# pangenome/poasta

Hardware: AMD Instinct MI355X
Metric: Gcells/sec (aligned bases/sec in config), gap-affine POA alignment, 1k-node POA x 10k x 1 kbp queries per GPU (higher is better)
Workload: dtype u16

## Files before the change

include/poasta_amd.h:

```cpp
#ifndef POASTA_AMD_H
#define POASTA_AMD_H

#include <stdint.h>

#ifdef __cplusplus
extern "C" {
#endif

#define POA_NONE 0xFFFFFFFFu
#define POA_SCORE_UNVISITED 0xFFFFFFFFu

#define POA_OK 0
#define POA_ERR_INVALID_ARG (-1)
#define POA_ERR_NOT_A_DAG (-2)
#define POA_ERR_NO_DEVICE (-3)
#define POA_ERR_HIP (-4)
#define POA_ERR_CAPACITY (-5)
#define POA_ERR_OUT_OF_MEMORY (-6)
#define POA_ERR_UNSUPPORTED (-7)

#define POA_FLAG_AMBIGUOUS 0x01u
#define POA_FLAG_START_QUIRK 0x02u
#define POA_FLAG_REF_PANIC 0x04u
#define POA_FLAG_SHORT_QUERY 0x08u
// ... 241 lines not shown
int poa_scoreset_workspace_bytes(poa_scoreset_t* s, uint64_t* bytes);
void poa_scoreset_destroy(poa_scoreset_t* s);
int poa_score_pairs(const poa_graph_t* const* graphs, uint32_t n_graphs, const poa_costs_t* costs, const poa_config_t* cfg,
                    uint32_t n_queries, const uint8_t* qseq, const uint64_t* qoff, uint64_t n_pairs, const uint32_t* pair_query,
                    const uint32_t* pair_graph, uint32_t* score, uint32_t* flags, poa_stats_t* stats, int device);
int poa_score_pairs_2piece(const poa_graph_t* const* graphs, uint32_t n_graphs, const poa_costs2_t* costs, const poa_config_t* cfg,
                           uint32_t n_queries, const uint8_t* qseq, const uint64_t* qoff, uint64_t n_pairs,
                           const uint32_t* pair_query, const uint32_t* pair_graph, uint32_t* score, uint32_t* flags,
                           poa_stats_t* stats, int device);

#ifdef __cplusplus
}
#endif
#include "poasta_amd_scoreset_cap.h"
#include "poasta_amd_scoreset_best.h"
#endif
```

poasta_amd/_lib.py:

```python
import ctypes as C
import os
import subprocess

_HERE = os.path.dirname(os.path.abspath(__file__))
LIB_PATH = os.environ.get("POA_LIB_PATH") or os.path.join(_HERE, "libpoasta_amd.so")
CSRC = os.path.join(_HERE, "csrc")

POA_OK = 0
ERRORS = {-1: "POA_ERR_INVALID_ARG", -2: "POA_ERR_NOT_A_DAG", -3: "POA_ERR_NO_DEVICE", -4: "POA_ERR_HIP",
          -5: "POA_ERR_CAPACITY", -6: "POA_ERR_OUT_OF_MEMORY", -7: "POA_ERR_UNSUPPORTED"}
POA_NONE = 0xFFFFFFFF
FLAG_AMBIGUOUS, FLAG_START_QUIRK, FLAG_REF_PANIC, FLAG_SHORT_QUERY, FLAG_TRUNCATED, FLAG_EMPTY_GRAPH = 1, 2, 4, 8, 16, 32
FLAG_CAPPED = 0x80

EXPORTS = ["poa_version", "poa_last_error", "poa_device_count", "poa_graph_create", "poa_graph_destroy",
           "poa_graph_rows", "poa_graph_node_rows", "poa_graph_update", "poa_align_batch", "poa_align_batch_ex", "poa_align_batch_2piece", "poa_align_batch_2piece_ex", "poa_planes_2piece", "poa_release_cache", "poa_batch_create", "poa_batch_run",
           "poa_batch_run_ex",
           "poa_batch_fetch", "poa_batch_stats", "poa_batch_device_results", "poa_batch_fetch_search_counters", "poa_batch_last_layout", "poa_batch_band_info", "poa_batch_band_pair_info", "poa_batch_band_narrow_info", "poa_batch_last_launch", "poa_batch_fetch_planes", "poa_batch_fetch_compact", "poa_batch_destroy",
           "poa_batch_run_2piece", "poa_batch_fetch_planes_2piece",
           "poa_graph_sweep_slots", "poa_batch_create_ex", "poa_batch_workspace_bytes", "poa_graph_checkpoint_plan", "poa_graph_checkpoint_plan2",
           "poa_multi_footprint", "poa_multi_create", "poa_multi_run", "poa_multi_fetch", "poa_multi_stats", "poa_multi_device_results",
           "poa_multi_workspace_bytes", "poa_multi_destroy", "poa_align_multi",
           "poa_multi_footprint_2piece", "poa_multi_create_2piece", "poa_multi_run_2piece", "poa_align_multi_2piece",
           "poa_scoreset_footprint", "poa_scoreset_create", "poa_scoreset_run", "poa_scoreset_run_2piece", "poa_scoreset_fetch",
           "poa_scoreset_stats", "poa_scoreset_device_results", "poa_scoreset_workspace_bytes", "poa_scoreset_destroy",
           "poa_score_pairs", "poa_score_pairs_2piece",
           "poa_graph_sweep_checks"]
EXPORTS_SCORESET_CAP = ["poa_scoreset_run_capped", "poa_scoreset_run_2piece_capped", "poa_scoreset_fetch_swept"]
EXPORTS_SCORESET_BEST = ["poa_scoreset_run_best", "poa_scoreset_run_2piece_best", "poa_scoreset_fetch_best", "poa_scoreset_device_best",
                         "poa_score_best", "poa_score_best_2piece"]
CFG_BEST_PAIR_ORDER = 2


class PoaBest(C.Structure):
    _fields_ = [("pair", C.c_uint32), ("score", C.c_uint32), ("flags", C.c_uint32), ("second_score", C.c_uint32),
                ("n_within", C.c_uint32), ("reserved", C.c_uint32 * 3)]


class PoaCosts2(C.Structure):
    _fields_ = [("mismatch", C.c_uint8), ("gap_open1", C.c_uint8), ("gap_extend1", C.c_uint8), ("gap_open2", C.c_uint8),
                ("gap_extend2", C.c_uint8), ("wide_planes", C.c_uint8), ("reserved", C.c_uint8 * 2)]


class PoaCosts(C.Structure):
    _fields_ = [("mismatch", C.c_uint8), ("gap_open", C.c_uint8), ("gap_extend", C.c_uint8), ("reserved", C.c_uint8)]

# ... 13 lines not shown
             "WS_CHUNK_CAP", "WS_PROF", "PS_LANES", "PS_LEAN", "TIMING", "WS_ADAPT", "WS_REC", "CKPT_ROWS", "BAND", "BAND_DELTA", "BAND_PAIR", "CAP_STRIDE")
EXACT_IMPLS = {"lane": 1, "wave": 2, "flat": 3}


def tune_from_env(cfg=None, **overrides):
    vals = {}
    for i, k in enumerate(TUNE_KEYS):
        v = overrides.get(k.lower(), os.environ.get("POA_" + k))
        if v is None or v == "":
            continue
        vals[i] = EXACT_IMPLS[v] if (k == "EXACT_IMPL" and v in EXACT_IMPLS) else int(v)
    nv = overrides.get("band_narrow", os.environ.get("POA_BAND_NARROW"))
    if nv is not None and nv != "":
        i = TUNE_KEYS.index("BAND_PAIR")
        vals[i] = (min(vals[i], 1) if i in vals else 2) | ((2 if int(nv) else 1) << 2)
    if cfg is None:
        if not vals:
            return None
        cfg = PoaConfig()
    for i, v in vals.items():
        cfg.tune[i] = v + 1
    return cfg


BOUND_UNBOUNDED, BOUND_INCLUDED, BOUND_EXCLUDED = 0, 1, 2
SPAN_GLOBAL, SPAN_ENDS_FREE = 0, 1


MODE_DENSE, MODE_EXACT, MODE_HYBRID, MODE_SCORE, MODE_CHECKPOINT, MODE_CHECKPOINT2 = 0, 1, 2, 3, 4, 5
HEURISTIC_DIJKSTRA, HEURISTIC_MINGAP = 0, 1
# ... 6 lines not shown
                ("n_chunks", C.c_uint32), ("n_forward_launches", C.c_uint32), ("n_flagged", C.c_uint32),
                ("ms_forward", C.c_float), ("ms_traceback", C.c_float), ("ms_h2d", C.c_float), ("ms_d2h", C.c_float),
                ("ms_exact", C.c_float), ("n_exact", C.c_uint32), ("ms_total", C.c_float), ("n_runs", C.c_uint32)]

    def as_dict(self):
        return {k: getattr(self, k) for k, _ in self._fields_ }


class PoaError(RuntimeError):
    def __init__(self, code, msg):
        super().__init__("%s (%d): %s" % (ERRORS.get(code, "POA_ERR"), code, msg))
        self.code = code


def build(force=False):
    srcs = [os.path.join(CSRC, f) for f in os.listdir(CSRC)] + [os.path.join(_HERE, "..", "include", h) for h in ("poasta_amd.h", "poasta_amd_scoreset_cap.h", "poasta_amd_scoreset_best.h")]
    stale = not os.path.exists(LIB_PATH) or any(os.path.getmtime(s) > os.path.getmtime(LIB_PATH) for s in srcs)
    if force or stale:
        subprocess.check_call(["make", "-C", CSRC] + (["-B"] if force else []))
    return LIB_PATH


_lib = None


def lib():
    global _lib
    if _lib is not None:
        return _lib
    if not os.path.exists(LIB_PATH):
        raise ImportError("poasta_amd: %s is missing — build it with `python -c 'import __graft_entry__ as g; g.build()'` "
# ... 70 lines not shown
    L.poa_batch_stats.restype = C.c_int
    L.poa_batch_stats.argtypes = [vp, C.POINTER(PoaStats)]
    L.poa_batch_fetch_search_counters.restype = C.c_int
    L.poa_batch_fetch_search_counters.argtypes = [vp, vp]
    L.poa_batch_last_layout.restype = C.c_int
    L.poa_batch_last_layout.argtypes = [vp, vp]
    if hasattr(L, "poa_batch_band_info"):
        L.poa_batch_band_info.restype = C.c_int
        L.poa_batch_band_info.argtypes = [vp, vp]
    if hasattr(L, "poa_batch_band_pair_info"):
        L.poa_batch_band_pair_info.restype = C.c_int
        L.poa_batch_band_pair_info.argtypes = [vp, vp]
    if hasattr(L, "poa_batch_band_narrow_info"):
        L.poa_batch_band_narrow_info.restype = C.c_int
        L.poa_batch_band_narrow_info.argtypes = [vp, vp]
    if hasattr(L, "poa_batch_last_launch"):
        L.poa_batch_last_launch.restype = C.c_int
        L.poa_batch_last_launch.argtypes = [vp, C.c_uint32, vp]
    L.poa_batch_device_results.restype = C.c_int
    L.poa_batch_device_results.argtypes = [vp, C.POINTER(vp), C.POINTER(vp), C.POINTER(vp), C.POINTER(vp)]
    L.poa_batch_fetch_planes.restype = C.c_int
    L.poa_batch_fetch_planes.argtypes = [vp, C.c_uint32, vp, vp, vp]
    if hasattr(L, "poa_batch_fetch_compact"):
        L.poa_batch_fetch_compact.restype = C.c_int
        L.poa_batch_fetch_compact.argtypes = [vp, C.c_uint32, vp, vp, vp]
    L.poa_batch_run_2piece.restype = C.c_int
    L.poa_batch_run_2piece.argtypes = [vp, C.POINTER(PoaCosts2), C.POINTER(PoaConfig), vp]
    L.poa_batch_fetch_planes_2piece.restype = C.c_int
    L.poa_batch_fetch_planes_2piece.argtypes = [vp, C.c_uint32, vp, vp, vp, vp, vp]
    L.poa_batch_destroy.argtypes = [vp]
# ... 63 lines not shown
```

poasta_amd/aligner.py:

```python
import ctypes as C
import os

import numpy as np

from . import _lib
from .graph import FlatGraph, pack_queries


class GapAffine:

    def __init__(self, cost_mismatch, cost_gap_extend, cost_gap_open):
        for v in (cost_mismatch, cost_gap_extend, cost_gap_open):
            if not 0 <= int(v) <= 255:
                raise ValueError("GapAffine costs are u8")
        self.cost_mismatch, self.cost_gap_extend, self.cost_gap_open = int(cost_mismatch), int(cost_gap_extend), int(cost_gap_open)

    def mismatch(self):
        return self.cost_mismatch

    def gap_open(self):
        return self.cost_gap_open

    def gap_extend(self):
        return self.cost_gap_extend
# ... 313 lines not shown

    def band_info(self):
        out = (C.c_uint32 * 4)()
        _lib.check(_lib.lib().poa_batch_band_info(self.handle, out))
        return {"used": bool(out[0]), "banded": int(out[1]), "fell_back": int(out[2]), "min_d": int(out[3])}

    def band_pair_info(self):
        out = (C.c_uint32 * 4)()
        _lib.check(_lib.lib().poa_batch_band_pair_info(self.handle, out))
        return {"paired": int(out[0]), "single": int(out[1]), "rule_count": int(out[2]), "ran_paired": bool(out[3])}

    def band_narrow_info(self):
        out = (C.c_uint32 * 4)()
        _lib.check(_lib.lib().poa_batch_band_narrow_info(self.handle, out))
        return {"ran": int(out[0]), "certified": int(out[1]), "certified_512": int(out[2]), "chosen_by": (None, "rule", "override")[int(out[3])]}

    def launches(self):
        out = []
        while True:
            v = (C.c_uint32 * 8)()
            rc = _lib.lib().poa_batch_last_launch(self.handle, len(out), v)
            if rc == -1 and (out or self.n == 0):
                return out
            _lib.check(rc)
            out.append({"kernel": LAUNCH_KERNELS[v[0]], "quads": int(v[1]), "fuse": bool(v[2] & 1), "mw": bool(v[2] & 2),
                        "waves": int(v[3]), "code_fmt": int(v[4]), "tb_lanes": int(v[5]), "tb_depth": int(v[6]), "queries": int(v[7])})

    def device_results(self):
        ptrs = [C.c_void_p() for _ in range(4)]
        _lib.check(_lib.lib().poa_batch_device_results(self.handle, *[C.byref(p) for p in ptrs]))
# ... 423 lines not shown
```

poasta_amd/csrc/poa_dense_plan.cpp:

```cpp
#include "poa_dense_plan.hpp"

#include <algorithm>

namespace poa_amd {

uint64_t score_bound(uint64_t open, uint64_t extend, uint64_t n_open, uint64_t n_extend) { return open * n_open + extend * n_extend; }
bool u16_cells_suffice(uint64_t open, uint64_t extend, uint64_t n_open, uint64_t n_extend) {
    return score_bound(open, extend, n_open, n_extend) <= 65534;
}
bool planes32(const TuneView& T) { const int* pv = T.ptr(POA_TUNE_PLANES); return pv && *pv == 32; }

uint32_t mw_waves(uint32_t strips) {
    const uint32_t groups = (strips + DENSE_MW_MAX_WAVES - 1) / DENSE_MW_MAX_WAVES;
    return (strips + groups - 1) / groups;
}

bool pxmw_ok(const TuneView& T, uint32_t count, uint32_t max_pitch) {
    if (const int* v = T.ptr(POA_TUNE_PXMW)) return (*v) != 0;
    return (uint64_t)count * ((max_pitch + 1023) / 1024) >= 1024;
}

DenseRunPlan plan_dense_run(uint32_t gap_open, uint32_t gap_extend, uint64_t max_len, uint64_t min_path_nodes, uint32_t mode, bool want_full,
                            bool plan16_same, const TuneView& T) {
    DenseRunPlan R;
// ... 13 lines not shown
    R.plan = (R.narrow && mode == POA_MODE_DENSE && !plan16_same) ? (R.compact ? 2 : 1) : 0;
    R.spec_depth = 12;
    if (const int* sv = T.ptr(POA_TUNE_TB_DEPTH)) { const int v = (*sv); if (v >= 1 && v <= 64) R.spec_depth = (uint32_t)v; }
    R.tb_group = 0;
    if (const int* gv = T.ptr(POA_TUNE_TB_GROUP)) { const int v = (*gv); if (v == 8 || v == 16 || v == 32 || v == 64) R.tb_group = v; }
    R.fuse_tb = false;
    if (const int* fv = T.ptr(POA_TUNE_FUSE_TB)) R.fuse_tb = (*fv) != 0;
    R.quads_override = 0;
    if (const int* ov = T.ptr(POA_TUNE_FWD_QUADS)) R.quads_override = (*ov);
    R.want_band = mode == POA_MODE_DENSE && gap_extend > 0;
    if (const int* bv = T.ptr(POA_TUNE_BAND)) R.want_band = R.want_band && (*bv) != 0;
    R.band_cap = 0xFFFFFFFFu;
    if (const int* dv = T.ptr(POA_TUNE_BAND_DELTA)) R.band_cap = (*dv) > 0 ? (uint32_t)(*dv) : 0u;
    R.band_pair = -1;
    R.band_narrow = -1;
    if (const int* pv = T.ptr(POA_TUNE_BAND_PAIR)) {
        const int p = (*pv) & POA_BAND_PAIR_MASK, n = ((*pv) >> POA_BAND_NARROW_SHIFT) & 3;
        if (p != POA_BAND_PAIR_RULE) R.band_pair = p != 0 ? 1 : 0;
        if (n) R.band_narrow = n - 1;
    }
    return R;
}

constexpr uint32_t BAND_NARROW_MIN_SHARE = 4;
uint32_t band_narrow_class(uint32_t d_n, uint32_t L) {
    if (d_n < 4) return 2;
    return (uint64_t)BAND_NARROW_MIN_SHARE * (d_n - 4) >= L ? 0 : 1;
}
uint32_t band_narrow_pairs(const DenseRunPlan& R, bool pair_by_rule, uint32_t n_rule, uint32_t n_any) {
    if (R.band_narrow == 0) return 0;
    if (R.band_narrow > 0) return n_any;
    return pair_by_rule ? n_rule : 0;
}

DenseChunkPlan plan_dense_chunk(const DenseRunPlan& R, uint32_t count, uint32_t max_pitch, const TuneView& T) {
    uint32_t lk = POA_KERNEL_NONE, lq = 0, lwaves = 4, code_fmt = 0;
    bool lfuse = false, lmw = false;
    int mf = -1;
    const int quads_override = R.quads_override;
    if (R.narrow) {
        uint32_t quads = max_pitch <= 512 ? 1 : 2;
        if (quads_override == 1 || quads_override == 2) quads = (uint32_t)quads_override;
        if (R.relative) quads = 2;
        lk = R.compact && R.packed ? POA_KERNEL_PACKED : POA_KERNEL_FORWARD; lq = quads;
        if (R.compact && R.packed) {
            bool mw = max_pitch > 512 * quads;
            if (const int* mv = T.ptr(POA_TUNE_MW)) mw = mw && ((*mv) != 0 || R.relative);
            bool px = max_pitch <= 1024 && quads == 2 && (!R.fuse_tb || R.relative);
            if (const int* xv = T.ptr(POA_TUNE_PX)) px = (px && (*xv) != 0) || (px && R.relative);
            if (px) {
// ... 19 lines not shown
        if (mw) {
            const uint32_t s2 = (max_pitch + 511) / 512, s4 = (max_pitch + 1023) / 1024;
            const uint32_t g2 = (s2 + DENSE_MW_MAX_WAVES - 1) / DENSE_MW_MAX_WAVES, g4 = (s4 + 9) / 10;
            bool wide = 14 * g4 < 10 * g2 || (uint64_t)count * s4 >= 8192;
            if (quads_override == 4) wide = true;
            if (quads_override == 2) wide = false;
            lq = wide ? 4 : 2; lmw = true; lwaves = wide ? (s4 + g4 - 1) / g4 : (s2 + g2 - 1) / g2;
        } else lfuse = R.fuse_tb;
    }
    uint32_t ltb = 0, ldepth = R.spec_depth;
    if (!(R.fuse_tb && !R.relative && max_pitch <= 1024 && (!R.compact || R.packed))) {
        const int tbg = R.tb_group ? R.tb_group : (count <= 6144 ? 64 : (count <= 12288 ? 32 : 16));
        ltb = R.compact ? (uint32_t)tbg : 64u;
        if (R.compact && !T.ptr(POA_TUNE_TB_DEPTH)) ldepth = tbg == 16 ? 16u : 32u;
    }
    return {{lk, lq, (lfuse ? POA_LAUNCH_FUSE : 0u) | (lmw ? POA_LAUNCH_MW : 0u), lwaves, code_fmt, ltb, ldepth, count}, mf, lk == POA_KERNEL_BAND, ltb != 0};
}

}
```

poasta_amd/csrc/poa_dense_plan.hpp:

```cpp
#pragma once
#include <cstdint>

#include "../../include/poasta_amd.h"

struct TuneView {
    int val[POA_TUNE_COUNT]; bool set[POA_TUNE_COUNT];
    explicit TuneView(const poa_config_t* cfg) { for (int k = 0; k < POA_TUNE_COUNT; ++k) { set[k] = cfg && cfg->tune[k] != 0; val[k] = set[k] ? (int)cfg->tune[k] - 1 : 0; } }
    const int* ptr(int k) const { return set[k] ? &val[k] : nullptr; }
};

namespace poa_amd {
constexpr uint32_t DENSE_MW_MAX_WAVES = 16;
uint64_t score_bound(uint64_t open, uint64_t extend, uint64_t n_open, uint64_t n_extend);
bool u16_cells_suffice(uint64_t open, uint64_t extend, uint64_t n_open, uint64_t n_extend);
bool planes32(const TuneView& T);
uint32_t mw_waves(uint32_t strips);
bool pxmw_ok(const TuneView& T, uint32_t count, uint32_t max_pitch);

struct DenseRunPlan {
    uint64_t ub;
    bool narrow, compact, relative, packed;
    int plan;
    bool fuse_tb, want_band;
    int quads_override, band_pair, tb_group;
    int band_narrow;
    uint32_t band_cap, spec_depth;
};
DenseRunPlan plan_dense_run(uint32_t gap_open, uint32_t gap_extend, uint64_t max_len, uint64_t min_path_nodes, uint32_t mode, bool full_planes,
                            bool plan16_same, const TuneView& T);

struct DenseChunkPlan {
    uint32_t v[8];
    int mf;
    bool band;
    bool separate_tb;
};
DenseChunkPlan plan_dense_chunk(const DenseRunPlan& R, uint32_t count, uint32_t max_pitch, const TuneView& T);
uint32_t band_narrow_class(uint32_t d_n, uint32_t L);
uint32_t band_narrow_pairs(const DenseRunPlan& R, bool pair_by_rule, uint32_t n_rule, uint32_t n_any);
}
```

poasta_amd/csrc/poa_engine.hip:

```cpp
#include <hip/hip_runtime.h>

#include <algorithm>
#include <array>
#include <chrono>
#include <cstdio>
#include <cstdlib>
#include <cstring>
#include <map>
#include <memory>
#include <new>
#include <mutex>
#include <string>
#include <vector>

#include "../../include/poasta_amd.h"
#include "poa_graph.hpp"
#include "poa_exact_kernel.hpp"
#include "poa_wsearch.hpp"
#include "poa_fsearch.hpp"

#include "poa_dense_plan.hpp"
#include "poa_kernels.hpp"
#include "poa_forward_packed.hpp"
#include "poa_forward_px.hpp"
#include "poa_band_plan.hpp"
#include "poa_forward_band.hpp"
#include "poa_twopiece.hpp"
#include "poa_sweep_rows.hpp"
#include "poa_forward_sweep.hpp"
#include "poa_checkpoint.hpp"
#include "poa_checkpoint2.hpp"
#include "poa_multi_plan.hpp"
#include "poa_multi.hpp"
#include "poa_scoreset_plan.hpp"
#include "poa_scoreset.hpp"

using namespace poa_amd;
// ... 194 lines not shown
    CheckpointPlan ckpt_plan;
    uint32_t ckpt_slots = 0;
    bool ckpt2 = false;
    DevBuf<uint32_t> d_ck_snap_off, d_ck_snap_dst, d_ck_pred_src, d_ck_boundary;

    bool band_ready = false;
    uint32_t band_n_seg = 0;
    std::vector<uint32_t> h_band_cls, h_band_d;
    DevBuf<uint32_t> d_band_cls, d_band_d, d_band_base;
    DevBuf<uint32_t> d_band_list, d_band_count;
    std::vector<uint32_t> h_band_dn;
    DevBuf<uint32_t> d_band_dn, d_band_base_n, d_band_list_n;
    std::vector<uint32_t> h_band_order;
    std::vector<uint32_t> h_band_nnarrow_rule, h_band_nnarrow_any;
    uint32_t narrow_ran = 0, narrow_how = 0, narrow_chunks = 0;
    int band_pair_plan = -1;
    std::vector<uint32_t> h_band_npair;
    DevBuf<uint32_t> d_band_order;
    uint32_t pair_paired = 0, pair_single = 0;
    bool band_used = false;
    uint32_t band_queries = 0, band_min_d = 0, band_chunks = 0;
    std::vector<DenseChunkPlan> launches;

    std::vector<std::vector<hipEvent_t>> runs;
    std::vector<std::vector<hipEvent_t>> free_sets;
    bool ran = false;
    hipStream_t last_stream = nullptr;
    float ms_h2d = 0.f;

    ~poa_batch() {
// ... 348 lines not shown
    HIP_TRY(hipGetLastError());
    hipLaunchKernelGGL(poa_forward_band_kernel<true>, dim3(blocks), dim3(256), 0, stream, fp, bp);
    uint32_t min_d = 0xFFFFFFFFu;
    for (uint32_t i = ch.first; i < ch.first + ch.count; ++i) min_d = std::min(min_d, std::min(b->h_band_d[b->h_band_cls[i]], R.band_cap));
    for (uint32_t k = 0; k < 2 * n_narrow; ++k) min_d = std::min(min_d, std::min(b->h_band_dn[b->h_band_cls[b->h_band_order[ch.first + k]]], R.band_cap));
    b->band_min_d = b->band_used ? std::min(b->band_min_d, min_d) : min_d;
    b->band_used = true; b->band_queries += ch.count; b->band_chunks = (uint32_t)ci + 1;
    return POA_OK;
}

void launch_traceback(const DenseRunPlan& R, const DenseChunkPlan& c, const TbParams& tp, hipStream_t stream) {
    const uint32_t lanes = c.v[5], per_block = 256 / lanes;
    const dim3 grid((c.v[7] + per_block - 1) / per_block), block(256);
    TbParams tpg = tp;
    tpg.spec_depth = c.v[6];
    if (R.compact && lanes == 16) hipLaunchKernelGGL((poa_traceback_kernel<uint16_t, true, 16>), grid, block, 0, stream, tpg);
    else if (R.compact && lanes == 32) hipLaunchKernelGGL((poa_traceback_kernel<uint16_t, true, 32>), grid, block, 0, stream, tpg);
    else if (R.compact && lanes == 8) hipLaunchKernelGGL((poa_traceback_kernel<uint16_t, true, 8>), grid, block, 0, stream, tpg);
    else if (R.compact) hipLaunchKernelGGL((poa_traceback_kernel<uint16_t, true>), grid, block, 0, stream, tpg);
    else if (R.narrow) hipLaunchKernelGGL((poa_traceback_kernel<uint16_t, false>), grid, block, 0, stream, tp);
    else hipLaunchKernelGGL((poa_traceback_kernel<uint32_t, false>), grid, block, 0, stream, tp);
}

template <typename SearchParams>
void fill_search_params(SearchParams& sp, poa_batch* b, const ExactParams& ep, const TuneView& T) {
    sp.E = ep;
    sp.chunks = reinterpret_cast<ExU4*>(b->d_ex_pool.p);
    sp.chunk_cap = b->ex_pool_cap / BQ_CHUNK;
    if (const int* cv = T.ptr(POA_TUNE_WS_CHUNK_CAP)) { const int v = (*cv); if (v >= 1 && (uint32_t)v < sp.chunk_cap) sp.chunk_cap = (uint32_t)v; }
    sp.win = b->ex_win;
    sp.counters = b->d_ex_counters.p;
// ... 721 lines not shown
        if (rc != POA_OK) return rc;
    }
    RunFrame run;
    if (const int rc = run.open(b, "poa_batch_run: call poa_batch_stats/fetch at least every 256 runs")) return rc;
    const DenseRunPlan R = plan_dense_run(costs->gap_open, costs->gap_extend, b->max_len, fg.min_path_nodes, mode,
                                          cfg && (cfg->flags & POA_CFG_FULL_PLANES), b->plan16_same, T);
    if (const int rc = run.begin(stream, b->plan[R.plan].chunks.size())) return rc;
    b->prof_on = T.ptr(POA_TUNE_WS_PROF) != nullptr;
    b->last_mode = mode;
    b->two_piece = false;
    set_layout(b, R.narrow, R.compact, R.relative);
    b->launches.clear();
    b->band_used = false; b->band_queries = 0; b->band_min_d = 0; b->band_chunks = 0;
    b->pair_paired = 0; b->pair_single = 0;
    b->narrow_ran = 0; b->narrow_how = 0; b->narrow_chunks = 0;
    b->active_plan = R.plan;
    const poa_batch::Plan& PL = b->cur();
    if (b->n_queries == 0) return run.end_empty(true);
    if (R.want_band && !PL.chunks.empty()) {
        if (b->d_band_count.n < 3 * PL.chunks.size()) HIP_TRY(b->d_band_count.alloc(3 * PL.chunks.size()));
        HIP_TRY(hipMemsetAsync(b->d_band_count.p, 0, 3 * PL.chunks.size() * 4, stream));
    }
    for (size_t ci = 0; ci < PL.chunks.size(); ++ci) {
        const auto& ch = PL.chunks[ci];
        uint32_t max_pitch = 0;
        for (uint32_t i = ch.first; i < ch.first + ch.count; ++i) max_pitch = std::max(max_pitch, b->h_pitch[i]);
        const DenseChunkPlan C = plan_dense_chunk(R, ch.count, max_pitch, T);
        TbParams tp;
        tp.rows = b->d_rows.p; tp.pred_rows = b->d_pred_rows.p; tp.n_rows = fg.n;
        tp.start_row = fg.start_row; tp.end_row = fg.end_row;
        tp.first_query = ch.first; tp.n_queries = ch.count;
        tp.qseq = b->d_qseq.p; tp.qoff = b->d_qoff.p; tp.pitch = b->d_pitch.p; tp.plane_off = PL.d_off.p;
        tp.planes = b->d_planes.p; tp.scratch_off = b->d_scratch_off.p; tp.scratch = b->d_scratch.p;
        tp.score = b->d_score.p; tp.flags = b->d_flags.p; tp.n_pairs = b->d_npairs.p;
        tp.cost_x = costs->mismatch; tp.cost_o = costs->gap_open; tp.cost_e = costs->gap_extend;
        tp.spec_depth = R.spec_depth;
        tp.exact_pass = 0; tp.ex_status = nullptr; tp.ex_end = nullptr; tp.code_fmt = C.v[4];
        tp.row_depth = R.relative ? b->d_row_depth.p : nullptr;
        tp.d_slot = fg.d_slot.empty() ? nullptr : b->d_dslot.p; tp.pred_dslot = fg.d_slot.empty() ? nullptr : b->d_pred_dslot.p;
        FwdParams fp;
        fp.rows = b->d_rows.p; fp.pred_rows = b->d_pred_rows.p; fp.n_rows = fg.n;
        fp.first_query = ch.first; fp.n_queries = ch.count;
// ... 4 lines not shown
        fp.cost_doe = R.relative ? (uint32_t)costs->gap_open : fp.cost_oe;
        fp.cost_ie = R.relative ? 2u * fp.cost_e : fp.cost_e;
        fp.cost_ioe = R.relative ? fp.cost_oe + fp.cost_e : fp.cost_oe;
        fp.pred_k = R.relative ? b->d_pred_k.p : nullptr;
        fp.d_slot = fg.d_slot.empty() ? nullptr : b->d_dslot.p; fp.pred_dslot = fg.d_slot.empty() ? nullptr : b->d_pred_dslot.p;
        fp.pipeline_error = b->d_pipeline_error.p;
        if (C.mf >= 0) b->dense_derived_gaps = C.mf == 3;
        if (C.band) { if (const int rc = launch_band(b, ci, R, fp, stream)) return rc; }
        else launch_forward(R, C, fp, tp, stream);
        HIP_TRY(hipGetLastError());
        if (const int rc = run.mark()) return rc;

        if (C.separate_tb) {
            launch_traceback(R, C, tp, stream);
            HIP_TRY(hipGetLastError());
        }
        if (mode == POA_MODE_DENSE) b->launches.push_back(C);
        if (const int rc = run.mark()) return rc;

        if (mode != POA_MODE_DENSE) {
            if (const int rc = replay_chunk(b, ch, costs, cfg, T, mode == POA_MODE_HYBRID ? 1u : 0u, ends_free, tp, stream)) return rc;
        }
        if (const int rc = run.mark()) return rc;
    }
    return run.end_pairs();
}

int poa_batch_fetch(poa_batch_t* b, uint32_t* score, poa_aln_pair_t* pairs, uint64_t* pair_off, uint64_t pair_capacity,
                    uint32_t* flags, poa_stats_t* stats) {
    if (!b) return fail(POA_ERR_INVALID_ARG, "poa_batch_fetch: null batch");
// ... 129 lines not shown
}

int poa_batch_band_narrow_info(poa_batch_t* b, uint32_t out[4]) {
    if (!b || !out) return fail(POA_ERR_INVALID_ARG, "poa_batch_band_narrow_info: null argument");
    if (!b->ran) return fail(POA_ERR_INVALID_ARG, "poa_batch_band_narrow_info: poa_batch_run has not been called");
    out[0] = b->narrow_ran; out[1] = 0; out[2] = 0; out[3] = b->narrow_how;
    if (!b->narrow_ran) return POA_OK;
    HIP_TRY(hipSetDevice(b->device));
    HIP_TRY(hipStreamSynchronize(b->last_stream));
    const size_t n_chunks = b->cur().chunks.size();
    std::vector<uint32_t> counts(3 * n_chunks);
    HIP_TRY(hipMemcpy(counts.data(), b->d_band_count.p, counts.size() * 4, hipMemcpyDeviceToHost));
    uint32_t missed = 0, missed_both = 0;
    for (size_t c = 0; c < n_chunks; ++c) { missed += counts[n_chunks + c]; missed_both += counts[2 * n_chunks + c]; }
    out[1] = b->narrow_ran - std::min(missed, b->narrow_ran); out[2] = missed - std::min(missed_both, missed);
    return POA_OK;
}

int poa_batch_band_pair_info(poa_batch_t* b, uint32_t out[4]) {
    if (!b || !out) return fail(POA_ERR_INVALID_ARG, "poa_batch_band_pair_info: null argument");
    if (!b->ran) return fail(POA_ERR_INVALID_ARG, "poa_batch_band_pair_info: poa_batch_run has not been called");
    out[0] = b->pair_paired; out[1] = b->pair_single; out[2] = BAND_PAIR_MIN_QUERIES; out[3] = b->pair_paired ? 1u : 0u;
    return POA_OK;
}

int poa_batch_fetch_planes(poa_batch_t* b, uint32_t query, uint32_t* m, uint32_t* i, uint32_t* d) {
    if (!b || !m || !i || !d) return fail(POA_ERR_INVALID_ARG, "poa_batch_fetch_planes: null argument");
    if (!b->ran || query >= b->n_queries) return fail(POA_ERR_INVALID_ARG, "poa_batch_fetch_planes: bad query / not run");
    if (b->compact) return fail(POA_ERR_UNSUPPORTED, "poa_batch_fetch_planes: the last run used the compact layout; run with POA_CFG_FULL_PLANES");
    if (b->sweep) return fail(POA_ERR_UNSUPPORTED, "poa_batch_fetch_planes: a score-only batch keeps no score planes");
// ... 1597 lines not shown
```

Before: 2841.

## Add lean traceback kernel specialized for compact u16 MF-coded planes

```diff
diff --git a/include/poasta_amd.h b/include/poasta_amd.h
--- a/include/poasta_amd.h
+++ b/include/poasta_amd.h
@@ -279,4 +279,5 @@
 #endif
 #include "poasta_amd_scoreset_cap.h"
 #include "poasta_amd_scoreset_best.h"
+#include "poasta_amd_tb.h"
 #endif
diff --git a/include/poasta_amd_tb.h b/include/poasta_amd_tb.h
--- /dev/null
+++ b/include/poasta_amd_tb.h
@@ -0,0 +1,19 @@
+#ifndef POASTA_AMD_TB_H
+#define POASTA_AMD_TB_H
+#include "poasta_amd.h"
+#ifdef __cplusplus
+extern "C" {
+#endif
+
+#define POA_TB_LEAN_SHIFT 4
+enum {
+    POA_TB_KERNEL_NONE = 0,
+    POA_TB_KERNEL_GENERIC,
+    POA_TB_KERNEL_LEAN
+};
+int poa_batch_tb_info(poa_batch_t* b, uint32_t out[4]);
+
+#ifdef __cplusplus
+}
+#endif
+#endif
diff --git a/poasta_amd/_lib.py b/poasta_amd/_lib.py
--- a/poasta_amd/_lib.py
+++ b/poasta_amd/_lib.py
@@ -30,6 +30,8 @@
 EXPORTS_SCORESET_BEST = ["poa_scoreset_run_best", "poa_scoreset_run_2piece_best", "poa_scoreset_fetch_best", "poa_scoreset_device_best",
                          "poa_score_best", "poa_score_best_2piece"]
 CFG_BEST_PAIR_ORDER = 2
+EXPORTS_TB = ["poa_batch_tb_info"]
+TB_LEAN_SHIFT = 4
 
 
 class PoaBest(C.Structure):
@@ -73,6 +75,10 @@
     if nv is not None and nv != "":
         i = TUNE_KEYS.index("BAND_PAIR")
         vals[i] = (min(vals[i], 1) if i in vals else 2) | ((2 if int(nv) else 1) << 2)
+    lv = overrides.get("tb_lean", os.environ.get("POA_TB_LEAN"))
+    if lv is not None and lv != "":
+        i = TUNE_KEYS.index("BAND_PAIR")
+        vals[i] = (vals[i] if i in vals else 2) | ((2 if int(lv) else 1) << TB_LEAN_SHIFT)
     if cfg is None:
         if not vals:
             return None
@@ -109,7 +115,7 @@
 
 
 def build(force=False):
-    srcs = [os.path.join(CSRC, f) for f in os.listdir(CSRC)] + [os.path.join(_HERE, "..", "include", h) for h in ("poasta_amd.h", "poasta_amd_scoreset_cap.h", "poasta_amd_scoreset_best.h")]
+    srcs = [os.path.join(CSRC, f) for f in os.listdir(CSRC)] + [os.path.join(_HERE, "..", "include", h) for h in ("poasta_amd.h", "poasta_amd_scoreset_cap.h", "poasta_amd_scoreset_best.h", "poasta_amd_tb.h")]
     stale = not os.path.exists(LIB_PATH) or any(os.path.getmtime(s) > os.path.getmtime(LIB_PATH) for s in srcs)
     if force or stale:
         subprocess.check_call(["make", "-C", CSRC] + (["-B"] if force else []))
@@ -210,6 +216,9 @@
     if hasattr(L, "poa_batch_band_narrow_info"):
         L.poa_batch_band_narrow_info.restype = C.c_int
         L.poa_batch_band_narrow_info.argtypes = [vp, vp]
+    if hasattr(L, "poa_batch_tb_info"):
+        L.poa_batch_tb_info.restype = C.c_int
+        L.poa_batch_tb_info.argtypes = [vp, vp]
     if hasattr(L, "poa_batch_last_launch"):
         L.poa_batch_last_launch.restype = C.c_int
         L.poa_batch_last_launch.argtypes = [vp, C.c_uint32, vp]
diff --git a/poasta_amd/aligner.py b/poasta_amd/aligner.py
--- a/poasta_amd/aligner.py
+++ b/poasta_amd/aligner.py
@@ -351,6 +351,11 @@
         out = (C.c_uint32 * 4)()
         _lib.check(_lib.lib().poa_batch_band_narrow_info(self.handle, out))
         return {"ran": int(out[0]), "certified": int(out[1]), "certified_512": int(out[2]), "chosen_by": (None, "rule", "override")[int(out[3])]}
+
+    def tb_info(self):
+        out = (C.c_uint32 * 4)()
+        _lib.check(_lib.lib().poa_batch_tb_info(self.handle, out))
+        return {"kernel": (None, "generic", "lean")[int(out[0])], "lanes": int(out[1]), "depth": int(out[2]), "walks": int(out[3])}
 
     def launches(self):
         out = []
diff --git a/poasta_amd/csrc/poa_dense_plan.cpp b/poasta_amd/csrc/poa_dense_plan.cpp
--- a/poasta_amd/csrc/poa_dense_plan.cpp
+++ b/poasta_amd/csrc/poa_dense_plan.cpp
@@ -51,12 +51,19 @@
     if (const int* dv = T.ptr(POA_TUNE_BAND_DELTA)) R.band_cap = (*dv) > 0 ? (uint32_t)(*dv) : 0u;
     R.band_pair = -1;
     R.band_narrow = -1;
+    R.tb_lean = -1;
     if (const int* pv = T.ptr(POA_TUNE_BAND_PAIR)) {
-        const int p = (*pv) & POA_BAND_PAIR_MASK, n = ((*pv) >> POA_BAND_NARROW_SHIFT) & 3;
+        const int p = (*pv) & POA_BAND_PAIR_MASK, n = ((*pv) >> POA_BAND_NARROW_SHIFT) & 3, l = ((*pv) >> POA_TB_LEAN_SHIFT) & 3;
         if (p != POA_BAND_PAIR_RULE) R.band_pair = p != 0 ? 1 : 0;
         if (n) R.band_narrow = n - 1;
+        if (l == 1 || l == 2) R.tb_lean = l - 1;
     }
+    R.tb_lean_mode = mode == POA_MODE_DENSE;
     return R;
+}
+
+bool tb_lean_eligible(const DenseRunPlan& R, uint32_t tb_lanes, uint32_t code_fmt, uint64_t plane_elems) {
+    return R.tb_lean_mode && tb_lanes != 0 && R.compact && code_fmt == 4 && !R.relative && plane_elems < (1ull << 32);
 }
 
 constexpr uint32_t BAND_NARROW_MIN_SHARE = 4;
@@ -70,7 +77,7 @@
     return pair_by_rule ? n_rule : 0;
 }
 
-DenseChunkPlan plan_dense_chunk(const DenseRunPlan& R, uint32_t count, uint32_t max_pitch, const TuneView& T) {
+DenseChunkPlan plan_dense_chunk(const DenseRunPlan& R, uint32_t count, uint32_t max_pitch, const TuneView& T, uint64_t plane_elems) {
     uint32_t lk = POA_KERNEL_NONE, lq = 0, lwaves = 4, code_fmt = 0;
     bool lfuse = false, lmw = false;
     int mf = -1;
@@ -120,7 +127,8 @@
         ltb = R.compact ? (uint32_t)tbg : 64u;
         if (R.compact && !T.ptr(POA_TUNE_TB_DEPTH)) ldepth = tbg == 16 ? 16u : 32u;
     }
-    return {{lk, lq, (lfuse ? POA_LAUNCH_FUSE : 0u) | (lmw ? POA_LAUNCH_MW : 0u), lwaves, code_fmt, ltb, ldepth, count}, mf, lk == POA_KERNEL_BAND, ltb != 0};
+    const bool lean = R.tb_lean != 0 && tb_lean_eligible(R, ltb, code_fmt, plane_elems);
+    return {{lk, lq, (lfuse ? POA_LAUNCH_FUSE : 0u) | (lmw ? POA_LAUNCH_MW : 0u), lwaves, code_fmt, ltb, ldepth, count}, mf, lk == POA_KERNEL_BAND, ltb != 0, lean};
 }
 
 }
diff --git a/poasta_amd/csrc/poa_dense_plan.hpp b/poasta_amd/csrc/poa_dense_plan.hpp
--- a/poasta_amd/csrc/poa_dense_plan.hpp
+++ b/poasta_amd/csrc/poa_dense_plan.hpp
@@ -25,6 +25,8 @@
     int quads_override, band_pair, tb_group;
     int band_narrow;
     uint32_t band_cap, spec_depth;
+    int tb_lean;
+    bool tb_lean_mode;
 };
 DenseRunPlan plan_dense_run(uint32_t gap_open, uint32_t gap_extend, uint64_t max_len, uint64_t min_path_nodes, uint32_t mode, bool full_planes,
                             bool plan16_same, const TuneView& T);
@@ -34,8 +36,10 @@
     int mf;
     bool band;
     bool separate_tb;
+    bool lean_tb;
 };
-DenseChunkPlan plan_dense_chunk(const DenseRunPlan& R, uint32_t count, uint32_t max_pitch, const TuneView& T);
+DenseChunkPlan plan_dense_chunk(const DenseRunPlan& R, uint32_t count, uint32_t max_pitch, const TuneView& T, uint64_t plane_elems = ~0ull);
+bool tb_lean_eligible(const DenseRunPlan& R, uint32_t tb_lanes, uint32_t code_fmt, uint64_t plane_elems);
 uint32_t band_narrow_class(uint32_t d_n, uint32_t L);
 uint32_t band_narrow_pairs(const DenseRunPlan& R, bool pair_by_rule, uint32_t n_rule, uint32_t n_any);
 }
diff --git a/poasta_amd/csrc/poa_engine.hip b/poasta_amd/csrc/poa_engine.hip
--- a/poasta_amd/csrc/poa_engine.hip
+++ b/poasta_amd/csrc/poa_engine.hip
@@ -21,6 +21,7 @@
 
 #include "poa_dense_plan.hpp"
 #include "poa_kernels.hpp"
+#include "poa_traceback_mf.hpp"
 #include "poa_forward_packed.hpp"
 #include "poa_forward_px.hpp"
 #include "poa_band_plan.hpp"
@@ -245,6 +246,7 @@
     std::vector<uint32_t> h_band_order;
     std::vector<uint32_t> h_band_nnarrow_rule, h_band_nnarrow_any;
     uint32_t narrow_ran = 0, narrow_how = 0, narrow_chunks = 0;
+    uint32_t tb_kernel = 0, tb_lanes = 0, tb_depth = 0, tb_walks = 0;
     int band_pair_plan = -1;
     std::vector<uint32_t> h_band_npair;
     DevBuf<uint32_t> d_band_order;
@@ -623,7 +625,11 @@
     const dim3 grid((c.v[7] + per_block - 1) / per_block), block(256);
     TbParams tpg = tp;
     tpg.spec_depth = c.v[6];
-    if (R.compact && lanes == 16) hipLaunchKernelGGL((poa_traceback_kernel<uint16_t, true, 16>), grid, block, 0, stream, tpg);
+    if (c.lean_tb && lanes == 16) hipLaunchKernelGGL((poa_traceback_mf_kernel<16>), grid, block, 0, stream, tpg);
+    else if (c.lean_tb && lanes == 32) hipLaunchKernelGGL((poa_traceback_mf_kernel<32>), grid, block, 0, stream, tpg);
+    else if (c.lean_tb && lanes == 8) hipLaunchKernelGGL((poa_traceback_mf_kernel<8>), grid, block, 0, stream, tpg);
+    else if (c.lean_tb) hipLaunchKernelGGL((poa_traceback_mf_kernel<64>), grid, block, 0, stream, tpg);
+    else if (R.compact && lanes == 16) hipLaunchKernelGGL((poa_traceback_kernel<uint16_t, true, 16>), grid, block, 0, stream, tpg);
     else if (R.compact && lanes == 32) hipLaunchKernelGGL((poa_traceback_kernel<uint16_t, true, 32>), grid, block, 0, stream, tpg);
     else if (R.compact && lanes == 8) hipLaunchKernelGGL((poa_traceback_kernel<uint16_t, true, 8>), grid, block, 0, stream, tpg);
     else if (R.compact) hipLaunchKernelGGL((poa_traceback_kernel<uint16_t, true>), grid, block, 0, stream, tpg);
@@ -1375,6 +1381,7 @@
     b->band_used = false; b->band_queries = 0; b->band_min_d = 0; b->band_chunks = 0;
     b->pair_paired = 0; b->pair_single = 0;
     b->narrow_ran = 0; b->narrow_how = 0; b->narrow_chunks = 0;
+    b->tb_kernel = POA_TB_KERNEL_NONE; b->tb_lanes = 0; b->tb_depth = 0; b->tb_walks = 0;
     b->active_plan = R.plan;
     const poa_batch::Plan& PL = b->cur();
     if (b->n_queries == 0) return run.end_empty(true);
@@ -1386,7 +1393,7 @@
         const auto& ch = PL.chunks[ci];
         uint32_t max_pitch = 0;
         for (uint32_t i = ch.first; i < ch.first + ch.count; ++i) max_pitch = std::max(max_pitch, b->h_pitch[i]);
-        const DenseChunkPlan C = plan_dense_chunk(R, ch.count, max_pitch, T);
+        const DenseChunkPlan C = plan_dense_chunk(R, ch.count, max_pitch, T, compact_plane_elems(fg.n, max_pitch, fg.d_slot.empty() ? fg.n : fg.n_store_d));
         TbParams tp;
         tp.rows = b->d_rows.p; tp.pred_rows = b->d_pred_rows.p; tp.n_rows = fg.n;
         tp.start_row = fg.start_row; tp.end_row = fg.end_row;
@@ -1421,6 +1428,9 @@
         if (C.separate_tb) {
             launch_traceback(R, C, tp, stream);
             HIP_TRY(hipGetLastError());
+            if (!C.lean_tb) b->tb_kernel = POA_TB_KERNEL_GENERIC;
+            else if (b->tb_kernel == POA_TB_KERNEL_NONE) b->tb_kernel = POA_TB_KERNEL_LEAN;
+            b->tb_lanes = C.v[5]; b->tb_depth = C.v[6]; b->tb_walks += C.v[7];
         }
         if (mode == POA_MODE_DENSE) b->launches.push_back(C);
         if (const int rc = run.mark()) return rc;
@@ -1580,6 +1590,15 @@
     uint32_t missed = 0, missed_both = 0;
     for (size_t c = 0; c < n_chunks; ++c) { missed += counts[n_chunks + c]; missed_both += counts[2 * n_chunks + c]; }
     out[1] = b->narrow_ran - std::min(missed, b->narrow_ran); out[2] = missed - std::min(missed_both, missed);
+    return POA_OK;
+}
+
+int poa_batch_tb_info(poa_batch_t* b, uint32_t out[4]) {
+    if (!b || !out) return fail(POA_ERR_INVALID_ARG, "poa_batch_tb_info: null argument");
+    if (!b->ran) return fail(POA_ERR_INVALID_ARG, "poa_batch_tb_info: poa_batch_run has not been called");
+    const bool dense_family = !(b->two_piece || b->sweep || b->ckpt);
+    out[0] = dense_family ? b->tb_kernel : (uint32_t)POA_TB_KERNEL_NONE;
+    out[1] = dense_family ? b->tb_lanes : 0u; out[2] = dense_family ? b->tb_depth : 0u; out[3] = dense_family ? b->tb_walks : 0u;
     return POA_OK;
 }
 
diff --git a/poasta_amd/csrc/poa_traceback_mf.hpp b/poasta_amd/csrc/poa_traceback_mf.hpp
--- /dev/null
+++ b/poasta_amd/csrc/poa_traceback_mf.hpp
@@ -0,0 +1,339 @@
+#pragma once
+#include "poa_kernels.hpp"
+
+namespace poa_amd {
+
+struct MfCtx {
+    const RowMeta* rows;
+    const uint32_t* pred_rows;
+    const uint16_t* M;
+    const uint16_t* D;
+    const uint32_t* d_slot;
+    const uint32_t* pred_dslot;
+    const uint8_t* q;
+    uint32_t L, pitch, x, o, e;
+    __device__ __forceinline__ uint32_t raw(uint32_t row, uint32_t j) const { return (uint32_t)M[row * pitch + j]; }
+    __device__ __forceinline__ void cell(uint32_t row, uint32_t j, uint32_t& v, uint32_t& a, uint32_t& cf) const {
+        const uint32_t r = raw(row, j);
+        v = mf_value(r); a = (r >> 14) & 1u; cf = (r >> 15) & 1u;
+    }
+    __device__ __forceinline__ uint32_t m(uint32_t row, uint32_t j) const { return mf_value(raw(row, j)); }
+    __device__ __forceinline__ uint32_t d_at(uint32_t slot, uint32_t j) const { return PlaneIO<uint16_t>::widen((uint32_t)D[slot * pitch + j]); }
+    __device__ __forceinline__ uint32_t d_kept(uint32_t row, uint32_t j) const { return d_at(d_slot ? d_slot[row] : row, j); }
+    __device__ __forceinline__ uint32_t pred(uint32_t k) const { return pred_rows[k]; }
+    __device__ __forceinline__ uint32_t pred_d(uint32_t k, uint32_t j) const { return d_at(pred_dslot ? pred_dslot[k] : pred_rows[k], j); }
+};
+
+__device__ __forceinline__ void mf_cand(TbStep& f, uint32_t& n_cand, uint32_t row, uint32_t j, uint32_t st) {
+    if (!f.found) { f.row = row; f.j = j; f.st = st; f.found = true; }
+    n_cand++;
+}
+__device__ __forceinline__ uint32_t mf_sub(uint32_t a, uint32_t b, bool& panic) {
+    const uint32_t r = a - b;
+    if (r == INF) panic = true;
+    return r;
+}
+
+template <bool END>
+__device__ __forceinline__ TbStep mf_step_m(const MfCtx& c, const RowMeta& m, uint32_t row, uint32_t j, uint32_t raw, uint32_t up,
+                                            uint32_t& n_cand, bool& panic) {
+    TbStep f{0, 0, 0, false, 0, m.node};
+    n_cand = 0;
+    const uint32_t cs = mf_value(raw);
+    f.cs = cs;
+    if (cs == INF) return f;
+    if (j > 0) {
+        const bool moe = END || (uint32_t)m.sym == (uint32_t)c.q[j - 1];
+        const uint32_t pj = END ? j : j - 1;
+        const uint32_t target = (moe || m.pred_count == 0) ? cs : mf_sub(cs, c.x, panic);
+        if (!END && (m.flags & ROW_CHAIN)) {
+            if (up == target) mf_cand(f, n_cand, row - 1, pj, 0);
+        } else {
+            for (uint32_t k = 0; k < m.pred_count; ++k) {
+                const uint32_t pr = c.pred_rows[m.pred_begin + k];
+                if (c.m(pr, pj) == target) mf_cand(f, n_cand, pr, pj, 0);
+            }
+        }
+    }
+    if (raw & 0x8000u) mf_cand(f, n_cand, row, j, 1);
+    if (raw & 0x4000u) mf_cand(f, n_cand, row, j, 2);
+    return f;
+}
+__device__ __forceinline__ void mf_load_m(const MfCtx& c, uint32_t row, uint32_t j, uint32_t& raw, uint32_t& up) {
+    const uint32_t off = row * c.pitch + j;
+    raw = (uint32_t)c.M[off];
+    up = (row > 0 && j > 0) ? mf_value((uint32_t)c.M[off - c.pitch - 1u]) : INF;
+}
+
+template <bool END>
+__device__ __forceinline__ TbStep mf_step_d(const MfCtx& c, const RowMeta& m, uint32_t row, uint32_t j, uint32_t cs, uint32_t above,
+                                            uint32_t& n_cand, bool& bad, bool& panic) {
+    TbStep f{0, 0, 0, false, cs, m.node};
+    n_cand = 0;
+    if (cs == INF) return f;
+    if (m.pred_count == 0) return f;
+    const uint32_t t_open = mf_sub(mf_sub(cs, c.o, panic), c.e, panic), t_ext = mf_sub(cs, c.e, panic);
+    const bool is_end = END || (m.flags & ROW_END) != 0;
+    const bool real_open = !is_end && (j >= c.L || (uint32_t)m.sym != (uint32_t)c.q[j]);
+    if (m.flags & ROW_CHAIN) {
+        const uint32_t v = above;
+        if (v == t_open) mf_cand(f, n_cand, row - 1, j, 0);
+        else if (!real_open && v < t_open) bad = true;
+        if (tbd_d_extends(c, row, j, cs)) mf_cand(f, n_cand, row - 1, j, 1);
+    } else {
+        for (uint32_t k = 0; k < m.pred_count; ++k) {
+            const uint32_t pr = c.pred_rows[m.pred_begin + k];
+            const uint32_t v = c.m(pr, j);
+            if (v == t_open) mf_cand(f, n_cand, pr, j, 0);
+            else if (!real_open && v < t_open) bad = true;
+        }
+        for (uint32_t k = 0; k < m.pred_count; ++k)
+            if (c.pred_d(m.pred_begin + k, j) == t_ext) mf_cand(f, n_cand, c.pred_rows[m.pred_begin + k], j, 1);
+    }
+    return f;
+}
+
+__device__ __forceinline__ TbStep mf_step_i(const MfCtx& c, const RowMeta& m, uint32_t row, uint32_t j, uint32_t cs, uint32_t& n_cand,
+                                            bool& bad, bool& panic) {
+    TbStep f{0, 0, 0, false, cs, m.node};
+    n_cand = 0;
+    if (cs == INF) return f;
+    if (j > 0) {
+        const uint32_t t_open = mf_sub(mf_sub(cs, c.o, panic), c.e, panic), t_ext = mf_sub(cs, c.e, panic);
+        const uint32_t pm = c.m(row, j - 1);
+        if (pm == t_open) mf_cand(f, n_cand, row, j - 1, 0);
+        else if (!tbd_open_i(c, m, j - 1) && pm < t_open) bad = true;
+        if (tbd_i_extends(c, m, row, j, cs)) {
+            const bool only = (n_cand == 0);
+            mf_cand(f, n_cand, row, j - 1, 0);
+            if (only && pm != t_ext) bad = true;
+        }
+    }
+    return f;
+}
+
+template <int GW>
+__device__ __forceinline__ void traceback_mf_walk(const TbParams& P, const uint32_t qi, const uint32_t lane) {
+    const uint32_t gbase = (threadIdx.x & 63u) - lane;
+    auto gballot = [&](bool pred) -> uint64_t {
+        const uint64_t b = __ballot(pred);
+        if (GW == 64) return b;
+        const uint32_t w = (gbase & 32u) ? (uint32_t)(b >> 32) : (uint32_t)b;
+        return (uint64_t)((w >> (gbase & 31u)) & (uint32_t)((1ull << (GW & 63)) - 1ull));
+    };
+    auto ones = [](uint64_t b) -> uint32_t { return (b == ~0ull) ? 64u : (uint32_t)__builtin_ctzll(~b); };
+    auto bc = [&](uint32_t v, uint32_t src) { return (uint32_t)__shfl((int)v, (int)(gbase + src)); };
+
+    const uint64_t qbeg = P.qoff[qi];
+    MfCtx c;
+    c.rows = P.rows; c.pred_rows = P.pred_rows;
+    c.L = (uint32_t)(P.qoff[qi + 1] - qbeg);
+    c.q = P.qseq + qbeg;
+    c.pitch = P.pitch[qi];
+    const uint64_t RP = (uint64_t)P.n_rows * c.pitch;
+    c.M = reinterpret_cast<const uint16_t*>(P.planes) + P.plane_off[qi];
+    c.D = c.M + RP + RP / 4;
+    c.d_slot = P.d_slot; c.pred_dslot = P.pred_dslot;
+    c.x = P.cost_x; c.o = P.cost_o; c.e = P.cost_e;
+    const uint32_t L = c.L, start_row = P.start_row, end_row = P.end_row;
+
+    uint2* out = P.scratch + P.scratch_off[qi];
+    const uint32_t cap = (uint32_t)(P.scratch_off[qi + 1] - P.scratch_off[qi]);
+    uint32_t cnt = 0;
+    uint32_t flags = 0;
+    uint32_t lflags = 0;
+    auto emit_at = [&](uint32_t pos, uint32_t rpos, uint32_t qpos) {
+        if (pos < cap) out[cap - 1 - pos] = make_uint2(rpos, qpos);
+    };
+
+    if (lane == 0) P.score[qi] = c.m(end_row, L);
+    const uint32_t end_node = c.rows[end_row].node;
+
+    bool done = false;
+    uint32_t crow = 0, cj = 0, cst = 0;
+    uint32_t gcs = INF;
+    if (L == 0) done = true;
+    if (!done && L == 1) {
+        flags |= POA_FLAG_SHORT_QUERY;
+        if (lane == 0) emit_at(0, end_node, 0);
+        cnt = 1;
+        done = true;
+    }
+    if (!done) {
+        uint32_t f0 = 0, fr = 0, fj = 0, fs = 0, fallback = 0, fg = INF;
+        if (lane == 0) {
+            uint32_t nc; bool bad = false, pn = false;
+            const RowMeta me = c.rows[end_row];
+            TbStep cur = mf_step_m<true>(c, me, end_row, L, c.raw(end_row, L), INF, nc, pn);
+            fg = cur.cs;
+            if (cur.found && !pn && nc != 1) f0 |= POA_FLAG_AMBIGUOUS;
+            if (!cur.found && !pn) {
+                cur = mf_step_d<true>(c, me, end_row, L, c.d_kept(end_row, L), end_row > 0 ? c.m(end_row - 1, L) : INF, nc, bad, pn);
+                fg = cur.cs;
+                if (!pn) {
+                    if (!cur.found) { f0 |= POA_FLAG_REF_PANIC; fallback = 1; }
+                    else f0 |= POA_FLAG_AMBIGUOUS;
+                    if (cur.found && cur.st == 1) fg = cur.cs - c.e;
+                }
+            }
+            if (pn) { f0 |= POA_FLAG_REF_PANIC; fallback = 2; }
+            fr = cur.row; fj = cur.j; fs = cur.st;
+        }
+        flags |= bc(f0, 0);
+        const uint32_t fb = bc(fallback, 0);
+        if (fb) {
+            if (fb == 2) flags |= POA_FLAG_TRUNCATED;
+            if (fb == 1 && L <= 3) {
+                if (lane == 0) for (uint32_t i = 0; i < L; ++i) emit_at(i, end_node, L - 1 - i);
+                cnt = L;
+            }
+            done = true;
+        } else {
+            crow = bc(fr, 0); cj = bc(fj, 0); cst = bc(fs, 0); gcs = bc(fg, 0);
+        }
+    }
+    bool reached_start = done;
+    uint32_t d_run = 0, i_run = 0;
+    const uint32_t max_depth = P.spec_depth < (uint32_t)GW ? P.spec_depth : (uint32_t)GW;
+    while (!done) {
+        uint32_t depth = 1;
+        if (cst == 2 && crow != start_row && max_depth > 1 && cj > 1) {
+            uint32_t idepth = i_run < max_depth ? (i_run ? i_run : 1u) : max_depth;
+            if (idepth < 2) idepth = 2;
+            if (cj < idepth) idepth = cj;
+            const bool iact = lane < idepth;
+            const uint32_t jj = cj - lane;
+            TbStep sI{0, 0, 0, false, 0, 0}, sM{0, 0, 0, false, 0, 0};
+            uint32_t ncI = 0, ncM = 0;
+            bool badI = false, pnI = false, pnM = false;
+            RowMeta mi{};
+            if (iact) {
+                mi = c.rows[crow];
+                uint32_t rawL, upL;
+                mf_load_m(c, crow, jj - 1, rawL, upL);
+                const uint32_t gcs_i = lane == 0 ? gcs : c.m(crow, jj);
+                sI = mf_step_i(c, mi, crow, jj, gcs_i, ncI, badI, pnI);
+                if (sI.found && !pnI) sM = mf_step_m<false>(c, mi, crow, sI.j, rawL, upL, ncM, pnM);
+            }
+            const bool cyc = iact && sI.found && !pnI && sI.j + 1 == jj && sM.found && !pnM && sM.st == 2 && sM.row == crow && sM.j == sI.j;
+            const uint32_t ip = ones(gballot(cyc));
+            if (ip > 0) {
+                if (lane < ip) {
+                    if (ncI != 1 || badI || ncM != 1) lflags |= POA_FLAG_AMBIGUOUS;
+                    if (sI.j == 0 && (uint32_t)mi.sym == (uint32_t)c.q[0]) lflags |= POA_FLAG_START_QUIRK;
+                    emit_at(cnt + lane, POA_NONE, jj - 1);
+                }
+                cnt += ip;
+                cj -= ip;
+                gcs = bc(sM.cs, ip - 1);
+                i_run += ip;
+                continue;
+            }
+            const uint32_t w0 = bc(((sI.found && !pnI) ? 1u : 0u) | ((ncI != 1 || badI) ? 2u : 0u), 0);
+            if (w0 & 1u) {
+                if (w0 & 2u) flags |= POA_FLAG_AMBIGUOUS;
+                if (lane == 0) emit_at(cnt, POA_NONE, cj - 1);
+                cnt += 1;
+                const uint32_t n_row = crow, n_j = bc(sI.j, 0);
+                if (n_j == 0 && (uint32_t)c.rows[n_row].sym == (uint32_t)c.q[0]) flags |= POA_FLAG_START_QUIRK;
+                cj = n_j; cst = 0;
+                i_run = 0;
+                continue;
+            }
+        }
+        if (cst != 2) i_run = 0;
+        if (cst == 0) {
+            depth = max_depth;
+            if (crow + 1 < depth) depth = crow + 1;
+            if (cj + 1 < depth) depth = cj + 1;
+        } else if (cst == 1) {
+            depth = d_run < max_depth ? (d_run ? d_run : 1u) : max_depth;
+            if (crow + 1 < depth) depth = crow + 1;
+        }
+        if (cst != 1) d_run = 0;
+        const bool active = lane < depth;
+        const uint32_t my_row = crow - lane, my_j = (cst == 0) ? cj - lane : cj;
+        TbStep bt{0, 0, 0, false, 0, 0};
+        uint32_t nc = 0;
+        bool bad = false, pn = false;
+        if (active) {
+            const RowMeta m = c.rows[my_row];
+            if (cst == 0) {
+                uint32_t raw, up;
+                mf_load_m(c, my_row, my_j, raw, up);
+                bt = mf_step_m<false>(c, m, my_row, my_j, raw, up, nc, pn);
+            } else if (cst == 1) {
+                const uint32_t above = my_row > 0 ? c.m(my_row - 1, my_j) : INF;
+                bt = mf_step_d<false>(c, m, my_row, my_j, gcs - lane * c.e, above, nc, bad, pn);
+            } else bt = mf_step_i(c, m, my_row, my_j, gcs, nc, bad, pn);
+        }
+        const bool amb = active && bt.found && (nc != 1 || bad);
+        const bool quirk = active && bt.found && bt.st == 0 && bt.j == 0 && bt.row != start_row && cst != 1 &&
+                           (uint32_t)c.rows[bt.row].sym == (uint32_t)c.q[0];
+        const bool regular = active && bt.found && bt.row + 1 == my_row && bt.row != start_row &&
+                             ((cst == 0 && bt.st == 0 && bt.j + 1 == my_j) || (cst == 1 && bt.st == 1 && bt.j == my_j));
+        uint32_t p = ones(gballot(regular));
+        bool dies = false;
+        if (__ballot(active && pn)) {
+            const uint64_t pnb = gballot(active && pn);
+            const uint32_t first_pn = pnb ? (uint32_t)__builtin_ctzll(pnb) : 64u;
+            dies = pnb != 0 && first_pn <= p;
+            if (dies) p = first_pn;
+        }
+        if (lane < p) {
+            if (amb) lflags |= POA_FLAG_AMBIGUOUS;
+            if (quirk) lflags |= POA_FLAG_START_QUIRK;
+            emit_at(cnt + lane, bt.node, cst == 0 ? my_j - 1 : POA_NONE);
+        }
+        cnt += p;
+        if (dies) {
+            flags |= POA_FLAG_REF_PANIC;
+            break;
+        }
+        if (p == depth) {
+            crow -= depth;
+            if (cst == 0) cj -= depth;
+            else { gcs -= depth * c.e; d_run += depth; }
+            continue;
+        }
+        const uint32_t dw = bc((bt.found ? 1u : 0u) | (amb ? 2u : 0u) | (quirk ? 4u : 0u) | (bt.st << 3), p);
+        const uint32_t d_row = bc(bt.row, p), d_j = bc(bt.j, p), d_cs = bc(bt.cs, p), d_node = bc(bt.node, p);
+        const uint32_t d_st = dw >> 3;
+        const uint32_t cur_j = (cst == 0) ? cj - p : cj, cur_st = cst;
+        if (!(dw & 1u)) break;
+        if (dw & 2u) flags |= POA_FLAG_AMBIGUOUS;
+        if (cur_st == 0 && d_st != 0) {
+            crow = d_row; cj = d_j; cst = d_st;
+            gcs = d_cs;
+            continue;
+        }
+        if (lane == 0) {
+            if (cur_st == 0) emit_at(cnt, d_node, cur_j - 1);
+            else if (cur_st == 2) emit_at(cnt, POA_NONE, cur_j - 1);
+            else emit_at(cnt, d_node, POA_NONE);
+        }
+        cnt += 1;
+        if (dw & 4u) flags |= POA_FLAG_START_QUIRK;
+        if (d_row == start_row) { reached_start = true; break; }
+        if (cur_st == 1 && d_st == 1) gcs = d_cs - c.e;
+        if (cur_st == 1) d_run += p + 1;
+        crow = d_row; cj = d_j; cst = d_st;
+    }
+    if (!reached_start) flags |= POA_FLAG_TRUNCATED;
+    if (gballot((lflags & POA_FLAG_AMBIGUOUS) != 0)) flags |= POA_FLAG_AMBIGUOUS;
+    if (gballot((lflags & POA_FLAG_START_QUIRK) != 0)) flags |= POA_FLAG_START_QUIRK;
+    if (lane == 0) {
+        P.flags[qi] = flags;
+        P.n_pairs[qi] = cnt < cap ? cnt : cap;
+    }
+}
+
+template <int GW>
+__global__ __launch_bounds__(256) void poa_traceback_mf_kernel(TbParams P) {
+    const uint32_t lane = threadIdx.x & (uint32_t)(GW - 1);
+    const uint32_t wq = (blockIdx.x * blockDim.x + threadIdx.x) / (uint32_t)GW;
+    if (wq >= P.n_queries) return;
+    traceback_mf_walk<GW>(P, P.first_query + wq, lane);
+}
+
+}
```

After: 2984, median of 6. 1.05x the previous value.
